# winddori2002/DEX-TTS

Hardware: AMD Instinct MI355X
Metric: mel-frames/s at n_timesteps=50, 80-ch mel (sampler only); RTF (higher is better)
Workload: dtype bf16; 1 GPU; gedex_b1: gedex_lj B=1/GPU T=512 n_timesteps=50 (BASELINE.json configs[1]); global_batch=1, frames=512, hipgraph=False, parallelism=1 GPU

## Files before the change

dex_tts_amd/csrc/dex_api.hip:

```cpp
#include <hip/hip_runtime.h>
#include <cstdlib>

#include <cmath>
#include <cstdarg>
#include <atomic>
#include <cstdio>
#include <mutex>
#include <cstring>
#include <map>
#include <unordered_map>
#include <string_view>
#include <string>
#include <vector>

#include "../../include/dex_amd.h"
#include "kernels.h"
#include "weight_store.h"

using namespace dex;

namespace dex {
namespace {
const char* const KNOB_NAMES[] = {
    "DEX_CONV_STREAM", "DEX_CONV_PP", "DEX_CONV_SKIP_DEAD", "DEX_H_BF16", "DEX_ATTN_SEPARATE", "DEX_ATTN_Q64", "DEX_ATTN_Q64_TAIL", "DEX_ATTN_Q64_HALF", "DEX_DIT_XCDS", "DEX_ATTN_GENERIC", "DEX_RES2", "DEX_LP_INTER", "DEX_DIT_CHAIN",
    "DEX_DIT_CLUSTER", "DEX_DIT_CLUSTER_LOCAL", "DEX_ATTN_X_LP", "DEX_RES_X_LP", "DEX_CAT_LP", "DEX_XCD_MAP", "DEX_DEBUG_DROP_HANDOFF", "DEX_PATCH_FUSED",
    "DEX_CONV_DOWN", "DEX_CONVT_UP", "DEX_DEBUG_PLAN",
    "DEX_ATTN_SHARED_W8", "DEX_CONVT_MT", "DEX_CONVT_WGS", "DEX_CONV_DOWN_WGS", "DEX_CONV_REGW", "DEX_CONV_REGW_RES", "DEX_CONV_SMALL_MAX", "DEX_CONV_TH8",
    "DEX_CONV_W8", "DEX_DWCONV_CAP", "DEX_FINAL_CAP", "DEX_FIRST_CAP", "DEX_FIRST_MFMA", "DEX_GEMM_NWALK", "DEX_NWALK_SPLIT", "DEX_NWALK_BM", "DEX_POS_COL", "DEX_POS_COL_MIN",
    "DEX_POS_CT", "DEX_REGW_MIN_TILES", "DEX_REGW_WGS", "DEX_ROWCHAIN64", "DEX_ROWCHAIN64A", "DEX_TIV_CAP", "DEX_TV_CHAIN", "DEX_TIV_FOLD", "DEX_LINATTN_NSUB", "DEX_TV_FOLD", "DEX_OUT2_MIN", "DEX_NWALK_DMA",
    "DEX_LINATTN_HEADWAVES", "DEX_LINATTN_OUT2_HW", "DEX_CONV_ROUND1", "DEX_CONV_RESIDENT", "DEX_KVCTX_ROWS", "DEX_OUT2_ROWS", "DEX_PE_TOK", "DEX_NWALK_SMALL"};
constexpr int N_KNOBS = (int)(sizeof(KNOB_NAMES) / sizeof(KNOB_NAMES[0]));
int knob_parse(const char* e) {
    if (!e) return KNOB_UNSET;
    char* end = nullptr;
    const long v = strtol(e, &end, 10);
    if (end == e) {
        static bool warned = false;
        if (!warned) { warned = true; fprintf(stderr, "libdexamd: ignoring a DEX_* knob whose value '%s' is not an integer\n", e); }
        return KNOB_UNSET;
    }
    return (int)v;
}
struct KnobSnapshot {
    int v[N_KNOBS];
    KnobSnapshot() { for (int i = 0; i < N_KNOBS; ++i) v[i] = knob_parse(getenv(KNOB_NAMES[i])); }
};
thread_local const KnobSnapshot* t_knobs = nullptr;
struct WsplitScope {
    bool prev;
    explicit WsplitScope(bool on) : prev(g_lp_wsplit) { g_lp_wsplit = on; }
    ~WsplitScope() { g_lp_wsplit = prev; }
};
struct KnobScope {
    const KnobSnapshot* prev;
    explicit KnobScope(const KnobSnapshot* k) : prev(t_knobs) { t_knobs = k; }
    ~KnobScope() { t_knobs = prev; }
};
}
static int knob_index(const char* name) {
    static const std::unordered_map<std::string_view, int> idx = [] {
        std::unordered_map<std::string_view, int> m;
        for (int i = 0; i < N_KNOBS; ++i) m.emplace(KNOB_NAMES[i], i);
        return m;
// ... 506 lines not shown
        build_mel_constants(basis, filt);
        DEX_HIPCHK(x, hipMalloc((void**)&x->mel_basis, basis.size() * sizeof(float)));
        DEX_HIPCHK(x, hipMalloc((void**)&x->mel_filt, filt.size() * sizeof(float)));
        DEX_HIPCHK(x, hipMemcpy(x->mel_basis, basis.data(), basis.size() * sizeof(float), hipMemcpyHostToDevice));
        DEX_HIPCHK(x, hipMemcpy(x->mel_filt, filt.data(), filt.size() * sizeof(float), hipMemcpyHostToDevice));
    }
    if (x->alloc_rc != DEX_OK) return x->alloc_rc;
    DEX_HIPCHK(x, hipStreamSynchronize(st));
    DEX_HIPCHK(x, hipGetLastError());
    x->finalized = true;
    return DEX_OK;
}

namespace {

constexpr int SCAL_STRIDE = 8;
constexpr int LA_CHUNK = 512;
constexpr int POS_SPLIT = 8;

struct Dims { int B, T, Tr, Ts, n_steps; };

struct StageBuf {
    int H, W, C, mask_ws; long npix;
    float *h1, *a1, *h2, *rbuf, *r0out, *r1out;
    float *qkv, *pm, *ps, *pc, *weff, *ctxn; void* mbf; int nchunks, nblk_fused;
    float* attn_out; int attn_ld, attn_coff;
    float* ds_out;
};

struct Plan {
    Dims d;
    float *sig2, *scal, *t_unet, *t_dit, *tmp_u, *temb, *c_tmp, *c_emb, *fin_mod;
    std::vector<float*> tadd_down, tadd_up, ada;
    float *adap_tmp, *t_adap, *t_sty, *tv_k0, *tv_v0, *sap_m, *sap_s, *ref_mean, *ref_std;
    float *spk_tmp, *spk_plane;
    int* step; int* step_tab; gnfix_t* stats; long stats_bytes; int n_gn;
    float* xbuf;
    float *xprime, *dbuf, *hsig, *htab;
    float *that, *hstep, *ncoef;
    std::vector<StageBuf> down, up;
    std::vector<float*> cat;
    void* cat16;
    float *up_out, *hF;
    int Hm, Wm, Hf, Wt, N;
    float *pe0, *emb, *emb_pad, *pos_part, *tok, *xn, *qkv, *ao, *att_ml, *hmlp, *dbg_tok;
    float* xslab; unsigned* xflag; size_t xflag_bytes;
    int xlocal;
    void *qh, *kh, *vt, *qh2, *kh2, *vt2; int Npad; size_t vt_bytes;
    float *tv_keys, *tv_K, *tv_V, *tv_q, *tv_ao, *tv_out, *tiv_out, *tv_weff, *tv_beff; gnfix_t *tv_stats, *tiv_stats; void* tv_wbf;
    float* tiv_aff;
    void *tv_kp, *tv_vtp; int tv_nkpad;
    float *tv_G, *tv_Vp, *tv_g0, *tv_v0p, *tv_xmean;
    float* xin;
    size_t bytes;
};

__global__ __launch_bounds__(256) void zero_fill_kernel(uint4* p16, size_t n16, unsigned char* tail, int ntail) {
    const uint4 z = make_uint4(0u, 0u, 0u, 0u);
    for (size_t i = (size_t)blockIdx.x * 256 + threadIdx.x; i < n16; i += (size_t)gridDim.x * 256) p16[i] = z;
    if (blockIdx.x == 0 && (int)threadIdx.x < ntail) tail[threadIdx.x] = 0;
}
static void zero_fill(void* p, size_t bytes, hipStream_t st) {
    if (!p || !bytes) return;
    const size_t n16 = bytes / 16;
    size_t blocks = (n16 + 255) / 256; if (blocks > 1024) blocks = 1024; if (blocks < 1) blocks = 1;
    hipLaunchKernelGGL(zero_fill_kernel, dim3((unsigned)blocks), dim3(256), 0, st, reinterpret_cast<uint4*>(p), n16,
                       reinterpret_cast<unsigned char*>(p) + n16 * 16, (int)(bytes - n16 * 16));
// ... 25 lines not shown
    if (g_xcd_map.load(std::memory_order_acquire) >= 0) return;
    std::lock_guard<std::mutex> lk(g_xcd_probe_mutex);
    if (g_xcd_map.load(std::memory_order_relaxed) >= 0) return;
    if (knob_off("DEX_DIT_CLUSTER_LOCAL")) { g_xcd_map.store(0, std::memory_order_release); return; }
    unsigned* d = nullptr;
    if (hipMalloc(&d, 256 * sizeof(unsigned)) != hipSuccess) { (void)hipGetLastError(); g_xcd_map.store(0, std::memory_order_release); return; }
    bool ok = hipFuncSetAttribute(reinterpret_cast<const void*>(&xcc_probe_kernel), hipFuncAttributeMaxDynamicSharedMemorySize, 65536) == hipSuccess;
    unsigned h[256];
    for (int rep = 0; rep < 3 && ok; ++rep) {
        const int nb = rep == 0 ? 256 : rep == 1 ? 96 : 192;
        hipLaunchKernelGGL(xcc_probe_kernel, dim3(nb), dim3(512), 65536, 0, d);
        ok = hipMemcpy(h, d, nb * sizeof(unsigned), hipMemcpyDeviceToHost) == hipSuccess;
        for (int b = 8; b < nb && ok; ++b) ok = h[b] == h[b & 7];
    }
    hipFree(d);
    g_xcd_map.store(ok ? 1 : 0, std::memory_order_release);
}
extern "C" int dex_debug_xcd_local() { xcd_map_probe(); return g_xcd_map.load(); }

void make_plan(const DexCtx* x, const Dims& d, void* ws, Plan& P) {
    const DexConfig& c = x->cfg;
    Arena A; A.base = (char*)ws; A.dry = (ws == nullptr);
    A.trace = knob_set("DEX_DEBUG_PLAN") ? 1 : 0;
    P.d = d;
    const int n = d.n_steps, dim = c.dim, hid = c.dit_hidden, mid = mid_dim(c), B = d.B;
    P.sig2 = A.f(64);
    P.scal = A.f((size_t)n * SCAL_STRIDE); P.t_unet = A.f((size_t)n * dim); P.t_dit = A.f((size_t)n * 256);
    P.tmp_u = A.f((size_t)n * 4 * dim); P.temb = A.f((size_t)n * dim);
    P.c_tmp = A.f((size_t)n * hid); P.c_emb = A.f((size_t)n * hid); P.fin_mod = A.f((size_t)n * 2 * hid);
    P.tadd_down.clear(); P.tadd_up.clear(); P.ada.clear();
    for (int i = 0; i < c.n_stages; ++i) for (int r = 0; r < 2; ++r) P.tadd_down.push_back(A.f((size_t)n * stage_dim(c, i)));
    for (int j = 0; j < c.n_stages - 1; ++j) for (int r = 0; r < 2; ++r) P.tadd_up.push_back(A.f((size_t)n * stage_dim(c, c.n_stages - 2 - j)));
    for (int k = 0; k < c.dit_depth; ++k) P.ada.push_back(A.f((size_t)n * 6 * hid));
    P.adap_tmp = P.t_adap = P.t_sty = P.tv_k0 = P.tv_v0 = P.sap_m = P.sap_s = P.ref_mean = P.ref_std = nullptr;
    if (c.variant == DEX_VARIANT_DEX) {
        P.adap_tmp = A.f((size_t)n * dim); P.t_adap = A.f((size_t)n * 2 * dim); P.t_sty = A.f((size_t)n * 2 * dim);
        P.tv_k0 = A.f((size_t)n * mid); P.tv_v0 = A.f((size_t)n * mid);
        P.sap_m = A.f((size_t)n * B * mid); P.sap_s = A.f((size_t)n * B * mid);
        P.ref_mean = A.f((size_t)B * 8 * mid); P.ref_std = A.f((size_t)B * 8 * mid);
    }
    P.spk_tmp = P.spk_plane = nullptr;
    if (c.n_spks > 1) { P.spk_tmp = A.f((size_t)B * 4 * c.spk_emb_dim); P.spk_plane = A.f((size_t)B * c.n_feats); }
    P.step = (int*)A.take(256);
    P.step_tab = (int*)A.take((size_t)(n + 1) * sizeof(int));
    P.n_gn = 4 * c.n_stages + 4 * (c.n_stages - 1) + 1;
    P.stats_bytes = (long)P.n_gn * B * 8 * GN_SLOTS * 2 * sizeof(gnfix_t);
    P.stats = (gnfix_t*)A.take(2 * P.stats_bytes);
    P.xbuf = A.f((size_t)B * 80 * d.T);
    P.xprime = A.f((size_t)B * 80 * d.T); P.dbuf = A.f((size_t)B * 80 * d.T);
    P.hsig = A.f((size_t)n + 2); P.htab = A.f((size_t)n + 2);
    P.that = A.f((size_t)n + 2); P.hstep = A.f((size_t)n + 2); P.ncoef = A.f((size_t)n + 2);
    P.cat.assign(c.n_stages - 1, nullptr);
    P.cat16 = nullptr;
    if (c.n_stages == 2) P.cat16 = A.take((size_t)B * (c.n_feats >> 1) * (d.T >> 1) * 2 * stage_dim(c, 1) * 2);
    for (int j = 0; j < c.n_stages - 1; ++j) {
        const int i = c.n_stages - 1 - j;
        P.cat[j] = A.f((size_t)B * (c.n_feats >> i) * (d.T >> i) * 2 * stage_dim(c, i));
    }
    auto stage = [&](int H, int W, int C, int mws) {
        StageBuf s{};
        s.H = H; s.W = W; s.C = C; s.mask_ws = mws; s.npix = (long)H * W;
        const size_t e = (size_t)B * s.npix;
        s.h1 = A.f(e * C); s.a1 = A.f(e * C); s.h2 = A.f(e * C); s.rbuf = A.f(e * C); s.r0out = A.f(e * C); s.r1out = A.f(e * C);
        s.qkv = A.f(e * 384);
        s.nchunks = (int)((s.npix + LA_CHUNK - 1) / LA_CHUNK);
        s.nblk_fused = (int)((s.npix + 127) / 128);
        s.pm = A.f((size_t)B * 4 * s.nblk_fused * 32); s.ps = A.f((size_t)B * 4 * s.nblk_fused * 32);
        s.pc = A.f((size_t)B * 4 * s.nblk_fused * 1024); s.weff = A.f((size_t)B * 128 * C);
        s.ctxn = A.f((size_t)B * 4096); s.mbf = A.take((size_t)B * C * 128 * 2);
// ... 688 lines not shown
                    ConvTUpP u{};
                    u.X = s.attn_out; u.a_lp = g.a_lp; u.ldx = s.C; u.xb = (long)s.H * s.W * s.C; u.x_coff = 0; u.H = s.H; u.W = s.W;
                    for (int par = 0; par < 4; ++par) u.Wfrag[par] = x->up_us_w[j][par].frag[x->lpi()].p;
                    u.bias = x->up_us_b[j];
                    u.Y = dst; u.c_lp = g.c_lp; u.ldy = ldd; u.y_coff = 0;
                    u.inmask = mask; u.inmask_ws = s.mask_ws; u.mask_bstride = P.d.T; u.B = B;
                    const double M = 4.0 * s.H * s.W * B;
                    run("upsample_convT", 2.0 * M * s.C * 4 * s.C, M * s.C * (g.c_lp ? 2.0 : 4.0) + 0.25 * M * s.C * (g.a_lp ? 2.0 : 4.0),
                        [&] { launch_convt_up(u, x->precision, st); });
                } else gemm("upsample_convT", g);
            }
        }
        tap("up_out", P.up_out, (long)B * 80 * P.d.T, c.dim, c.dim);
        TD U{P.up_out, c.dim, 0, c.dim, up_out_lp ? lpk : 0};
        gnfix_t* stf = next_stats();
        const bool hfb = h_bf16() && fast_conv(c.dim, c.dim);
        conv3x3("conv3x3", U, 80, P.d.T, 1, true, x->fin_w, x->fin_b, c.dim, P.hF, stf, nullptr, nullptr, nullptr, false, hfb);
        FinalGP f{};
        f.x_bf16 = hfb ? x->lp_kind() : 0;
        f.X = P.hF; f.xb = 80L * P.d.T * c.dim; f.npix = 80 * P.d.T; f.W = P.d.T; f.C = c.dim; f.groups = 8; f.stats = stf;
        f.gamma = x->fin_g; f.beta = x->fin_be; f.mask = mask; f.mask_bstride = P.d.T; f.wfc = x->fconv_w; f.bfc = x->fconv_b;
        f.xcur = xcur; f.denoised = denoised; f.xnext = xnext; f.scal = P.scal; f.scal_stride = SCAL_STRIDE; f.step = sp; f.row_bstride = rbs; f.B = B;
        f.zero_ptr = reinterpret_cast<float*>(stats_other); f.zero_n = P.stats_bytes / (long)sizeof(float);
        f.poison = P.xflag ? reinterpret_cast<const int*>(P.xflag + (P.xflag_bytes - sizeof(int)) / sizeof(unsigned)) : nullptr;
        f.mode = up.mode; f.htab = up.htab; f.dbuf = P.dbuf; f.xhat = P.xbuf;
        f.gtab = up.gtab; f.xstate = up.xstate; f.xin_next = up.xin_next;
        FinalMP fm{};
        static_cast<FinalP&>(fm) = f;
        fm.mtab = up.mtab; fm.dprev_in = up.dprev_in; fm.dprev_out = up.dprev_out;
        run("final_conv_euler", 14.0 * 80 * P.d.T * c.dim * B, 80.0 * P.d.T * ((hfb ? 2.0 : 4.0) * c.dim + 12.0) * B,
            [&] { if (up.mtab) launch_final_multistep(fm, st); else if (up.gtab) launch_final_general(f, st); else launch_final(f, st); });
    }

    void prepare(const float* sigmas_dev, int n, bool levels = false) {
        const DexConfig& c = x->cfg;
        const int dim = c.dim, hid = c.dit_hidden, B = P.d.B, mid = mid_dim(c);
        auto R = [&](const std::string& k) { return x->raw.at(k).p; };
        auto lin = [&](const float* X, int ldx, int rows, int K, const std::string& w, bool bias, int N, float* Y, int ai, int ao) {
            SmallLinP s{X, ldx, rows, K, R(w + ".weight"), bias ? R(w + ".bias") : nullptr, N, Y, N, ai, ao};
            run("cond_mlp", 2.0 * rows * K * N, 4.0 * K * N, [&] { launch_small_linear(s, st); });
        };
        if (P.tv_stats) zero_fill(P.tv_stats, (size_t)B * mid_dim(c) * IN_SLOTS * 2 * 2 * sizeof(gnfix_t), st);
        if (P.xflag) zero_fill(P.xflag, P.xflag_bytes, st);
        zero_fill(P.vt, P.vt_bytes, st);
        zero_fill(P.vt2, P.vt_bytes, st);
        CondPrepP cp{sigmas_dev, n, c.pe_scale, dim, P.scal, SCAL_STRIDE, P.t_unet, P.t_dit, levels ? 1 : 0};
        run("cond_prep", 0, 0, [&] { launch_cond_prep(cp, st); });
        lin(P.t_unet, dim, n, dim, "mlp.0", true, 4 * dim, P.tmp_u, 0, 1);
        lin(P.tmp_u, 4 * dim, n, 4 * dim, "mlp.2", true, dim, P.temb, 0, 0);
        for (int i = 0; i < c.n_stages; ++i)
            for (int r = 0; r < 2; ++r)
                lin(P.temb, dim, n, dim, "downs." + std::to_string(i) + "." + std::to_string(r) + ".mlp.1", true, stage_dim(c, i), P.tadd_down[2 * i + r], 1, 0);
        for (int j = 0; j < c.n_stages - 1; ++j)
            for (int r = 0; r < 2; ++r)
                lin(P.temb, dim, n, dim, "ups." + std::to_string(j) + "." + std::to_string(r) + ".mlp.1", true, stage_dim(c, c.n_stages - 2 - j), P.tadd_up[2 * j + r], 1, 0);
        lin(P.t_dit, 256, n, 256, "vit.t_embedder.mlp.0", true, hid, P.c_tmp, 0, 2);
        lin(P.c_tmp, hid, n, hid, "vit.t_embedder.mlp.2", true, hid, P.c_emb, 0, 0);
        for (int k = 0; k < c.dit_depth; ++k)
            lin(P.c_emb, hid, n, hid, "vit.blocks." + std::to_string(k) + ".adaLN_modulation.1", true, 6 * hid, P.ada[k], 2, 0);
        lin(P.c_emb, hid, n, hid, "vit.final_layer.adaLN_modulation.1", true, 2 * hid, P.fin_mod, 2, 0);
        if (c.n_spks > 1) {
            lin(args->spk_dev, c.spk_emb_dim, B, c.spk_emb_dim, "spk_mlp.0", true, 4 * c.spk_emb_dim, P.spk_tmp, 0, 1);
            lin(P.spk_tmp, 4 * c.spk_emb_dim, B, 4 * c.spk_emb_dim, "spk_mlp.2", true, c.n_feats, P.spk_plane, 0, 0);
        }
        if (c.variant == DEX_VARIANT_DEX) {
            lin(P.t_unet, dim, n, dim, "mlp_adap.0", true, dim, P.adap_tmp, 0, 1);
            lin(P.adap_tmp, dim, n, dim, "mlp_adap.2", true, 2 * dim, P.t_adap, 0, 0);
            lin(P.t_unet, dim, n, dim, "mlp_adap_sty.0", true, dim, P.adap_tmp, 0, 1);
            lin(P.adap_tmp, dim, n, dim, "mlp_adap_sty.2", true, 2 * dim, P.t_sty, 0, 0);
            lin(P.t_sty, mid, n, mid, "tv_adaptor.w_k", false, mid, P.tv_k0, 0, 0);
            lin(P.t_sty, mid, n, mid, "tv_adaptor.w_v", false, mid, P.tv_v0, 0, 0);
            const int L = args->n_ref;
            for (int j = 0; j < L; ++j)
                run("ref_stats", 0, 4.0 * B * mid * args->Tr, [&] {
                    launch_row_stats(args->ref_skips_dev[j], B, mid, args->Tr, 1e-5f, P.ref_mean + (long)j * mid, P.ref_std + (long)j * mid, (long)L * mid, st);
                });
            SapP sm{P.t_adap, 2 * dim, 0, n, P.ref_mean, L, mid, R("tiv_adaptor.mean_sap.W.weight"), R("tiv_adaptor.mean_sap.W.bias"), P.sap_m, B};
            SapP ss{P.t_adap, 2 * dim, 0, n, P.ref_std, L, mid, R("tiv_adaptor.std_sap.W.weight"), R("tiv_adaptor.std_sap.W.bias"), P.sap_s, B};
            run("sap_pool", 0, 0, [&] { launch_sap(sm, st); launch_sap(ss, st); });
            run("sty_transpose", 0, 8.0 * B * mid * args->Ts, [&] { launch_transpose_cl(args->sty_dev, P.tv_keys, B, mid, args->Ts, 0, (long)args->Ts * mid, st); });
            for (int which = 0; which < 2; ++which) {
                float* dst = which ? P.tv_V : P.tv_K;
                IGemmP g = base_gemm(P.tv_keys, mid, 0, 1, args->Ts, mid, which ? x->tv_wv : x->tv_wk, mid, nullptr, dst + mid, mid, 0);
                g.c_bstride = (long)(args->Ts + 1) * mid;
                gemm("tv_kv", g);
            }
            if (tv_chain_on()) {
                TvKvPrepP kp{P.tv_K, P.tv_V, (long)(args->Ts + 1) * mid, args->Ts + 1, P.tv_nkpad, P.tv_kp, P.tv_vtp, B};
                run("tv_kv_operands", 0, 12.0 * B * (args->Ts + 1) * mid, [&] { launch_tv_kv_prep(kp, x->precision, st); });
            }
            if (tv_fold_on()) {
                const long kvb = (long)(args->Ts + 1) * mid;
                for (int which = 0; which < 2; ++which) {
                    IGemmP g = base_gemm((which ? P.tv_V : P.tv_K) + mid, mid, 0, 1, args->Ts, mid, which ? x->tv_wl.f32 : x->tv_wq_raw, mid, nullptr,
                                         (which ? P.tv_Vp : P.tv_G) + mid, mid, 0);
                    g.a_bstride = kvb; g.c_bstride = kvb;
                    gemm("tv_fold_kv", g);
                    IGemmP t = base_gemm(which ? P.tv_v0 : P.tv_k0, mid, 0, 1, n, mid, which ? x->tv_wl.f32 : x->tv_wq_raw, mid, nullptr, which ? P.tv_v0p : P.tv_g0, mid, 0);
                    t.B = 1;
                    gemm("tv_fold_time_rows", t);
                }
                TvKvPrepP kp{P.tv_G, P.tv_Vp, kvb, args->Ts + 1, P.tv_nkpad, P.tv_kp, P.tv_vtp, B};
                run("tv_fold_operands", 0, 6.0 * B * (args->Ts + 1) * mid, [&] { launch_tv_vfrag_prep(kp, x->precision, st); });
            }
// ... 40 lines not shown

struct SamplerKind {
    const DexSamplerTables* tb;
    bool heun, multistep, churn, scaled;
    int n, E;
    explicit SamplerKind(const DexSampleArgs* a)
        : tb(a->tables), heun(a->solver == DEX_SOLVER_HEUN), multistep(a->solver == DEX_SOLVER_DPMPP_2M), churn(tb ? (tb->flags & DEX_TABLES_CHURN) != 0 : a->S_churn > 0.f),
          scaled(tb && (tb->flags & DEX_TABLES_SCALED) != 0), n(a->n_steps), E(tb ? tb->n_rows : dex_num_evals(a->n_steps, a->solver)) {}

    Eval eval(const Plan& P, int e) const {
        if (multistep) return {P.xbuf, P.xbuf, {0, nullptr, nullptr, nullptr, nullptr, tb->coef_dev, e == 0 ? nullptr : P.dbuf, P.dbuf}, -1};
        const int i = heun ? e / 2 : e;
        const bool corrector = heun && (e & 1);
        const bool predictor = heun && !corrector && i < n - 1;
        const int mode = corrector ? 2 : predictor ? 1 : 0, noise_step = (churn && !corrector) ? i : -1;
        float* x = corrector ? P.xprime : P.xbuf;
        float* xout = predictor ? P.xprime : P.xbuf;
        if (!tb) return {x, xout, {mode, heun ? P.htab : churn ? P.hstep : nullptr}, noise_step};
        float* xin_next = (scaled && (predictor || (!churn && i < n - 1))) ? P.xin : nullptr;
        return {scaled ? P.xin : x, xout, {mode, nullptr, tb->coef_dev, x, xin_next}, noise_step};
    }
};

int enqueue_sampler(DexCtx* x, const DexSampleArgs* a, hipStream_t st) {
    const SamplerKind k(a);
    const DexSamplerTables* tb = k.tb;
    const int n = k.n, E = k.E;
    Plan P; Dims d{a->B, a->T, a->Tr, a->Ts, E};
    make_plan(x, d, a->workspace_dev, P);
    Runner R{x, P, st, a->mask_dev, a->mu_dev, P.xbuf, a, false};
    const long nx = (long)a->B * 80 * a->T;
    float* xin = k.scaled ? P.xin : nullptr;
    auto coef = [&](int e) { return tb->coef_dev + (long)e * DEX_TABLE_EVAL_COLS; };
    if (tb) {
        R.prepare(tb->sigma_dev, E);
    } else {
        if (k.heun || k.churn) launch_churn_tables(a->sigmas_dev, n, a->S_churn, a->S_min, a->S_max, a->S_noise, P.that, P.hstep, P.ncoef, st);
        if (k.heun) launch_heun_expand(P.that, P.hstep, n, P.hsig, P.htab, st);
        R.prepare(k.heun ? P.hsig : k.churn ? P.that : a->sigmas_dev, E);
    }
    R.run("init_scale", 0, 8.0 * nx, [&] {
        if (tb) launch_ablation_init(a->z_dev, P.xbuf, tb->step_dev + 2, k.churn ? nullptr : xin, coef(0) + 1, nx, st);
        else launch_scale_copy(a->z_dev, P.xbuf, nx, a->sigmas_dev, st);
    });
    gnfix_t* arena[2] = {P.stats, P.stats + P.stats_bytes / (long)sizeof(gnfix_t)};
    zero_fill(P.stats, 2 * P.stats_bytes, st);
    for (int e = 0; e < E; ++e) {
        const Eval ev = k.eval(P, e);
        const int i = ev.noise_step;
        R.sp = e; R.stats_base = arena[e & 1]; R.stats_other = arena[(e + 1) & 1];
        if (i >= 0 && tb)
            R.run("churn_noise", 3.0 * nx, 16.0 * nx, [&] {
                launch_ablation_churn(P.xbuf, a->noise_dev ? a->noise_dev + (long)i * nx : nullptr, tb->step_dev + (long)i * DEX_TABLE_STEP_COLS,
                                      xin, coef(e) + 1, nx, st);
            });
        else if (i >= 0)
            R.run("churn_noise", 2.0 * nx, 12.0 * nx, [&] { launch_add_noise(P.xbuf, a->noise_dev + (long)i * nx, P.ncoef + i, nx, st); });
        R.xcur = ev.xin; R.up = ev.up;
        R.step(nullptr, ev.xout);
    }
    R.run("copy_out", 0, 8.0 * nx, [&] { launch_scale_copy(P.xbuf, a->out_dev, nx, nullptr, st); });
    return DEX_OK;
}

struct CallScope {
    const KnobSnapshot knobs;
    const KnobScope knob_scope{&knobs};
    const WsplitScope wsplit_scope;
    explicit CallScope(DexCtx* x) : wsplit_scope(x->precision == DEX_PREC_FP16X2) { xcd_map_probe(); x->last_xerr = nullptr; }
};

std::vector<uint64_t> graph_key(const DexSampleArgs* a, int precision, hipStream_t st, const KnobSnapshot& knobs) {
    std::vector<uint64_t> key = {(uint64_t)a->B, (uint64_t)a->T, (uint64_t)a->Tr, (uint64_t)a->Ts, (uint64_t)a->n_steps, (uint64_t)a->solver,
                                 (uint64_t)precision, (uint64_t)a->n_ref, (uint64_t)(uintptr_t)st,
                                 (uint64_t)(uintptr_t)a->z_dev, (uint64_t)(uintptr_t)a->mu_dev, (uint64_t)(uintptr_t)a->mask_dev,
                                 (uint64_t)(uintptr_t)a->sigmas_dev, (uint64_t)(uintptr_t)a->spk_dev, (uint64_t)(uintptr_t)a->sty_dev,
                                 (uint64_t)(uintptr_t)a->sty_lengths_dev, (uint64_t)(uintptr_t)a->out_dev, (uint64_t)(uintptr_t)a->workspace_dev,
                                 (uint64_t)(uintptr_t)(a->S_churn > 0.f ? a->noise_dev : nullptr)};
    key.push_back((uint64_t)g_xcd_gen.load(std::memory_order_acquire));
// ... 300 lines not shown
```

dex_tts_amd/csrc/kernels.h:

```cpp
#pragma once
#include <hip/hip_runtime.h>
#include <stdint.h>

namespace dex {

constexpr int KNOB_UNSET = -2147483647 - 1;
int knob(const char* name);
inline int knob_or(const char* name, int dflt) { const int v = knob(name); return v == KNOB_UNSET ? dflt : v; }
inline bool knob_off(const char* name) { return knob(name) == 0; }
inline bool knob_set(const char* name) { return knob(name) != KNOB_UNSET; }
inline int device_cus() {
    static const int n = [] { int dev = 0, v = 0; (void)hipGetDevice(&dev); (void)hipDeviceGetAttribute(&v, hipDeviceAttributeMultiprocessorCount, dev); return v > 0 ? v : 256; }();
    return n;
}

constexpr int GN_SLOTS = 32;
typedef long long gnfix_t;

extern thread_local const char* g_last_symbol;

constexpr int PREC_FP32 = 0, PREC_BF16 = 1, PREC_FP16 = 2, PREC_FP16X2 = 3;
inline bool prec_wsplit(int precision) { return precision == PREC_FP16X2; }
extern thread_local bool g_lp_wsplit;
inline bool prec_is_lp(int precision) { return precision != PREC_FP32; }
// ... 224 lines not shown
                     int xcd_map;
                     int tail_g = 0, tail_ks = 0;
                     int half_g = 0, half_n = 0; };
void launch_attention_direct(const AttnDirectP& p, int precision, hipStream_t st);
bool attention_direct_batch_regime(int N, int B);
int attention_direct_ksplit(int N, int B);
void launch_attention_q64(const AttnDirectP& p, int precision, hipStream_t st);
int attention_q64_ksplit(int N, int B, int max_split);
void attention_q64_plan(int N, int B, int max_split, int* ks, int* tail_g, int* tail_ks);
bool attention_q64_half_plan(int N, int B, int* half_g, int* half_n);
void launch_dit_rowchain(const DitChainP& p, int precision, hipStream_t st);
void launch_pack_lp_frag(const float* src, void* dst, int K, int N, int precision, hipStream_t st);
void launch_pack_lp_frag_nk(const float* src, void* dst, int K, int N, int precision, hipStream_t st);

struct AttnP { const float* Q; int ldq; long qb; const float* K; int ldk; long kb; const float* V; int ldv; long vb;
               float* O; int ldo; long ob; int Nq, Nk; const int* kv_len; int kv_len_add; int heads; float scale; int B;
               int ksplit; long o_sstride; float* ml;
               long long* dbg;
               int head_dim;
               int force_generic;
               int o_lp; };
inline bool dit_sep64_small_n(int N, int B) {
    if (N < 512 || N >= 1024) return false;
    const long t = (long)B * ((N + 63) / 64), r = (t + 255) / 256;
    return t >= 256 && t * 100 >= r * 256 * 65;
}
bool attention_lp_shared_form(int Nq, int heads, int B, int ksplit);
bool attention_head_dim_supported(int hd);
void launch_attention(const AttnP& p, int precision, hipStream_t st);

struct SmallLinP { const float* X; int ldx; int rows; int K; const float* W; const float* bias; int N;
                   float* Y; int ldy; int act_in; int act_out; };
void launch_small_linear(const SmallLinP& p, hipStream_t st);

struct CondPrepP { const float* sigmas; int n; float pe_scale; int dim; float* scal; int scal_stride;
                   float* t_unet; float* t_dit;
                   int no_next = 0; };
void launch_cond_prep(const CondPrepP& p, hipStream_t st);

void launch_scale_copy(const float* src, float* dst, long n, const float* scal_ptr, hipStream_t st);
void launch_step_reset(int* step, hipStream_t st);
void launch_step_inc(int* step, hipStream_t st);
void launch_iota(int* dst, int n, hipStream_t st);
void launch_permute4(const float* src, float* dst, int d0, int d1, int d2, int d3, int p0, int p1, int p2, int p3,
                     hipStream_t st);
void launch_f32_residual_lp(const float* src, float* dst, long n, int precision, hipStream_t st);
void launch_f32_to_lp(const float* src, void* dst, long n, int precision, hipStream_t st);
void launch_pack_lp_nk(const float* src, void* dst, int K, int N, int precision, hipStream_t st);
void launch_spk_plane(const float* spk_out, float* plane, int B, int F, hipStream_t st);

void launch_row_stats(const float* X, int B, int C, int len, float eps, float* mean, float* std, long out_bstride, hipStream_t st);
constexpr int IN_SLOTS = GN_SLOTS;
struct InStatsP { const float* X; int ld; long bstride; int npix; int C; gnfix_t* stats; int B;
                  const float* mask; int mask_ws; long mask_bstride; int W; };
void launch_in_stats(const InStatsP& p, hipStream_t st);
struct SapP { const float* t_tok; int t_ld; int t_coff; int nsteps; const float* stats; int L; int C;
              const float* w; const float* bias; float* out; int B; };
void launch_sap(const SapP& p, hipStream_t st);
struct InFoldP { const gnfix_t* stats; int npix; float eps; const float* Wq; int C; float* Weff; float* beff; int B;
                 void* Wbf; int lp; int split = 0; };
void launch_in_fold(const InFoldP& p, hipStream_t st);
struct TivApplyP { const float* X; int ld; long xb; float* Y; int ldy; long yb; int npix; int C; const gnfix_t* stats;
                   float eps; const float* s_tab; const float* m_tab; int step; int B;
                   int row_bstride = 0; };
void launch_tiv_apply(const TivApplyP& p, hipStream_t st);
void launch_tiv_coef(const TivApplyP& p, float* aff, hipStream_t st);
struct TvRow0P { const float* k0; const float* v0; int step; float* K; float* V; long kvb; int C; int B;
                 float* zero_ptr; long zero_n;
                 void* Kp = nullptr; void* VTp = nullptr; int NkPad = 0; int lp_kind = 0;
                 int row_bstride = 0; };
void launch_tv_row0(const TvRow0P& p, hipStream_t st);
// ... 81 lines not shown
```

dex_tts_amd/csrc/unet_elem.hip:

```cpp
#include "kernels.h"
#include "bf16_util.h"
#include <cstdlib>

namespace dex {

__device__ __forceinline__ float mish_f(float x) {
    if (x > 20.f) return x;
    const float e = __expf(x);
    const float n = e * (e + 2.f);
    return x * (n * __builtin_amdgcn_rcpf(n + 2.f));
}
__device__ __forceinline__ float silu_f(float x) { return x * __builtin_amdgcn_rcpf(1.f + __expf(-x)); }


__device__ __forceinline__ void gn_mean_rstd(const gnfix_t* stats, int b, int groups, float* smean, float* srstd, int tid) {
    if (tid < groups * GN_SLOTS) {
        const int g = tid / GN_SLOTS;
        const longlong2 v = *reinterpret_cast<const longlong2*>(stats + (((long)b * groups + g) * GN_SLOTS + (tid % GN_SLOTS)) * 2);
        long long s1 = v.x, s2 = v.y;
        gn_slots_reduce<GN_SLOTS>(s1, s2);
        if ((tid % GN_SLOTS) == 0) gn_moments(s1, s2, 1e-5, smean[g], srstd[g]);
    }
}

// ... 595 lines not shown
    hipLaunchKernelGGL(final_kernel<FinalGP>, dim3((unsigned)final_blocks(p), p.B), dim3(256), 0, st, p);
}
__global__ void ablation_churn_kernel(float* x, const float* noise, const float* rk, float* xin, const float* s, long n) {
    const float r = rk[0], k = rk[1];
    const float sv = xin ? *s : 1.f;
    for (long i = (long)blockIdx.x * blockDim.x + threadIdx.x; i < n; i += (long)gridDim.x * blockDim.x) {
        float v = __fmul_rn(r, x[i]);
        if (noise) v = __fadd_rn(v, __fmul_rn(k, noise[i]));
        x[i] = v;
        if (xin) xin[i] = __fdiv_rn(v, sv);
    }
}
void launch_final_multistep(const FinalMP& p, hipStream_t st) {
    hipLaunchKernelGGL(final_kernel<FinalMP>, dim3((unsigned)final_blocks(p), p.B), dim3(256), 0, st, p);
}
void launch_ablation_churn(float* x, const float* noise, const float* rk, float* xin, const float* s, long n, hipStream_t st) {
    long blocks = (n + 255) / 256; if (blocks > 2048) blocks = 2048;
    hipLaunchKernelGGL(ablation_churn_kernel, dim3((unsigned)blocks), dim3(256), 0, st, x, noise, rk, xin, s, n);
}
__global__ void ablation_init_kernel(const float* z, float* x, const float* c0, float* xin, const float* s, long n) {
    const float c = *c0;
    const float sv = xin ? *s : 1.f;
    for (long i = (long)blockIdx.x * blockDim.x + threadIdx.x; i < n; i += (long)gridDim.x * blockDim.x) {
        const float v = __fmul_rn(z[i], c);
        x[i] = v;
        if (xin) xin[i] = __fdiv_rn(v, sv);
    }
}
void launch_ablation_init(const float* z, float* x, const float* c0, float* xin, const float* s, long n, hipStream_t st) {
    long blocks = (n + 255) / 256; if (blocks > 2048) blocks = 2048;
    hipLaunchKernelGGL(ablation_init_kernel, dim3((unsigned)blocks), dim3(256), 0, st, z, x, c0, xin, s, n);
}

__global__ void cond_prep_kernel(const CondPrepP p) {
    const int i = blockIdx.x;
    const int k = threadIdx.x;
    const float sigma = p.sigmas[i], sigma_next = p.no_next ? 0.f : p.sigmas[i + 1];
    const float sd = 0.5f;
    const float c_noise = logf(sigma) / 4.f;
    if (k == 0) {
        float* sc = p.scal + (long)i * p.scal_stride;
        const float s2 = sigma * sigma + sd * sd;
        sc[0] = sigma; sc[1] = sigma_next;
        sc[2] = 1.f / sqrtf(s2);
        sc[3] = __fmul_rn(__frcp_rn(s2), sd * sd);
        sc[4] = sigma * sd / sqrtf(s2);
        sc[5] = c_noise;
    }
    const int half = p.dim / 2;
    if (k < half) {
        const float e = (float)(log(10000.0) / (double)(half - 1));
        const float f = expf((float)k * -e);
        const float a = p.pe_scale * c_noise * f;
        p.t_unet[(long)i * p.dim + k] = sinf(a);
        p.t_unet[(long)i * p.dim + half + k] = cosf(a);
    }
    if (k < 128) {
        const float f = expf((float)(-log(10000.0)) * (float)k / 128.f);
        const float a = c_noise * f;
        p.t_dit[(long)i * 256 + k] = cosf(a);
        p.t_dit[(long)i * 256 + 128 + k] = sinf(a);
    }
}
void launch_cond_prep(const CondPrepP& p, hipStream_t st) {
    hipLaunchKernelGGL(cond_prep_kernel, dim3(p.n), dim3(128), 0, st, p);
}

__global__ __launch_bounds__(256) void small_linear_kernel(const SmallLinP p) {
    const int wave = (blockIdx.x * 256 + threadIdx.x) >> 6, lane = threadIdx.x & 63;
    if (wave >= p.N) return;
    const float* w = p.W + (long)wave * p.K;
    const float bias = p.bias ? p.bias[wave] : 0.f;
    const int r0 = blockIdx.y * 8;
    float acc[8];
#pragma unroll
    for (int j = 0; j < 8; ++j) acc[j] = 0.f;
    for (int k = lane; k < p.K; k += 64) {
        const float wk = w[k];
#pragma unroll
        for (int j = 0; j < 8; ++j) {
            const int r = min(r0 + j, p.rows - 1);
            float v = p.X[(long)r * p.ldx + k];
            if (p.act_in == 1) v = mish_f(v); else if (p.act_in == 2) v = silu_f(v);
            acc[j] = fmaf(v, wk, acc[j]);
        }
    }
#pragma unroll
    for (int j = 0; j < 8; ++j) {
        float a = acc[j];
        for (int o = 32; o > 0; o >>= 1) a += __shfl_xor(a, o);
        if (lane == 0 && r0 + j < p.rows) {
            float y = a + bias;
            if (p.act_out == 1) y = mish_f(y); else if (p.act_out == 2) y = silu_f(y);
            p.Y[(long)(r0 + j) * p.ldy + wave] = y;
        }
    }
}
void launch_small_linear(const SmallLinP& p, hipStream_t st) {
    hipLaunchKernelGGL(small_linear_kernel, dim3((p.N * 64 + 255) / 256, (p.rows + 7) / 8), dim3(256), 0, st, p);
}

__global__ void scale_copy_kernel(const float* src, float* dst, long n, const float* scal) {
    const float s = scal ? *scal : 1.f;
    for (long i = (long)blockIdx.x * blockDim.x + threadIdx.x; i < n; i += (long)gridDim.x * blockDim.x) dst[i] = src[i] * s;
}
void launch_scale_copy(const float* src, float* dst, long n, const float* scal_ptr, hipStream_t st) {
    long blocks = (n + 255) / 256; if (blocks > 2048) blocks = 2048;
    hipLaunchKernelGGL(scale_copy_kernel, dim3((unsigned)blocks), dim3(256), 0, st, src, dst, n, scal_ptr);
}
__global__ void iota_kernel(int* d, int n) { const int i = blockIdx.x * blockDim.x + threadIdx.x; if (i < n) d[i] = i; }
void launch_iota(int* dst, int n, hipStream_t st) { hipLaunchKernelGGL(iota_kernel, dim3((n + 255) / 256), dim3(256), 0, st, dst, n); }
__global__ void step_reset_kernel(int* s) { *s = 0; }
__global__ void step_inc_kernel(int* s) { *s = *s + 1; }
void launch_step_reset(int* step, hipStream_t st) { hipLaunchKernelGGL(step_reset_kernel, dim3(1), dim3(1), 0, st, step); }
void launch_step_inc(int* step, hipStream_t st) { hipLaunchKernelGGL(step_inc_kernel, dim3(1), dim3(1), 0, st, step); }

__global__ void permute4_kernel(const float* src, float* dst, int d0, int d1, int d2, int d3, int p0, int p1, int p2, int p3) {
    const long n = (long)d0 * d1 * d2 * d3;
    const int sd[4] = {d0, d1, d2, d3};
    const long ss[4] = {(long)d1 * d2 * d3, (long)d2 * d3, (long)d3, 1};
    const int pm[4] = {p0, p1, p2, p3};
    for (long i = (long)blockIdx.x * blockDim.x + threadIdx.x; i < n; i += (long)gridDim.x * blockDim.x) {
        long rem = i, off = 0;
        for (int a = 3; a >= 0; --a) {
            const int dim = sd[pm[a]];
            const int idx = (int)(rem % dim);
            rem /= dim;
            off += idx * ss[pm[a]];
        }
        dst[i] = src[off];
    }
}
// ... 42 lines not shown
```

Measured before the change: 29630 mel-frames/s.

## Batch conditioning MLP launches and fuse per-call zero-fills, cond prep, init scale

Conditioning linears in prepare() are grouped by dependency level and issued as one multi-job small-linear kernel per level, with weights held in registers when K<=256. The separate zero-fills, cond_prep and initial noise scaling are merged into a single call_begin kernel. This cuts the per-call launch count in the fixed setup before the sampler loop. A second scratch buffer keeps the two adaptor MLP chains from racing inside a level. The path is on by default and can be disabled with DEX_COND_BATCH.

Result: no change. 29670 mel-frames/s (median of 4 runs) (+0.1%).

```diff
diff --git a/dex_tts_amd/csrc/dex_api.hip b/dex_tts_amd/csrc/dex_api.hip
--- a/dex_tts_amd/csrc/dex_api.hip
+++ b/dex_tts_amd/csrc/dex_api.hip
@@ -28,7 +28,8 @@
     "DEX_ATTN_SHARED_W8", "DEX_CONVT_MT", "DEX_CONVT_WGS", "DEX_CONV_DOWN_WGS", "DEX_CONV_REGW", "DEX_CONV_REGW_RES", "DEX_CONV_SMALL_MAX", "DEX_CONV_TH8",
     "DEX_CONV_W8", "DEX_DWCONV_CAP", "DEX_FINAL_CAP", "DEX_FIRST_CAP", "DEX_FIRST_MFMA", "DEX_GEMM_NWALK", "DEX_NWALK_SPLIT", "DEX_NWALK_BM", "DEX_POS_COL", "DEX_POS_COL_MIN",
     "DEX_POS_CT", "DEX_REGW_MIN_TILES", "DEX_REGW_WGS", "DEX_ROWCHAIN64", "DEX_ROWCHAIN64A", "DEX_TIV_CAP", "DEX_TV_CHAIN", "DEX_TIV_FOLD", "DEX_LINATTN_NSUB", "DEX_TV_FOLD", "DEX_OUT2_MIN", "DEX_NWALK_DMA",
-    "DEX_LINATTN_HEADWAVES", "DEX_LINATTN_OUT2_HW", "DEX_CONV_ROUND1", "DEX_CONV_RESIDENT", "DEX_KVCTX_ROWS", "DEX_OUT2_ROWS", "DEX_PE_TOK", "DEX_NWALK_SMALL"};
+    "DEX_LINATTN_HEADWAVES", "DEX_LINATTN_OUT2_HW", "DEX_CONV_ROUND1", "DEX_CONV_RESIDENT", "DEX_KVCTX_ROWS", "DEX_OUT2_ROWS", "DEX_PE_TOK", "DEX_NWALK_SMALL",
+    "DEX_COND_BATCH"};
 constexpr int N_KNOBS = (int)(sizeof(KNOB_NAMES) / sizeof(KNOB_NAMES[0]));
 int knob_parse(const char* e) {
     if (!e) return KNOB_UNSET;
@@ -601,7 +602,7 @@
     Dims d;
     float *sig2, *scal, *t_unet, *t_dit, *tmp_u, *temb, *c_tmp, *c_emb, *fin_mod;
     std::vector<float*> tadd_down, tadd_up, ada;
-    float *adap_tmp, *t_adap, *t_sty, *tv_k0, *tv_v0, *sap_m, *sap_s, *ref_mean, *ref_std;
+    float *adap_tmp, *adap_tmp2, *t_adap, *t_sty, *tv_k0, *tv_v0, *sap_m, *sap_s, *ref_mean, *ref_std;
     float *spk_tmp, *spk_plane;
     int* step; int* step_tab; gnfix_t* stats; long stats_bytes; int n_gn;
     float* xbuf;
@@ -693,9 +694,9 @@
     for (int i = 0; i < c.n_stages; ++i) for (int r = 0; r < 2; ++r) P.tadd_down.push_back(A.f((size_t)n * stage_dim(c, i)));
     for (int j = 0; j < c.n_stages - 1; ++j) for (int r = 0; r < 2; ++r) P.tadd_up.push_back(A.f((size_t)n * stage_dim(c, c.n_stages - 2 - j)));
     for (int k = 0; k < c.dit_depth; ++k) P.ada.push_back(A.f((size_t)n * 6 * hid));
-    P.adap_tmp = P.t_adap = P.t_sty = P.tv_k0 = P.tv_v0 = P.sap_m = P.sap_s = P.ref_mean = P.ref_std = nullptr;
+    P.adap_tmp = P.adap_tmp2 = P.t_adap = P.t_sty = P.tv_k0 = P.tv_v0 = P.sap_m = P.sap_s = P.ref_mean = P.ref_std = nullptr;
     if (c.variant == DEX_VARIANT_DEX) {
-        P.adap_tmp = A.f((size_t)n * dim); P.t_adap = A.f((size_t)n * 2 * dim); P.t_sty = A.f((size_t)n * 2 * dim);
+        P.adap_tmp = A.f((size_t)n * dim); P.adap_tmp2 = A.f((size_t)n * dim); P.t_adap = A.f((size_t)n * 2 * dim); P.t_sty = A.f((size_t)n * 2 * dim);
         P.tv_k0 = A.f((size_t)n * mid); P.tv_v0 = A.f((size_t)n * mid);
         P.sap_m = A.f((size_t)n * B * mid); P.sap_s = A.f((size_t)n * B * mid);
         P.ref_mean = A.f((size_t)B * 8 * mid); P.ref_std = A.f((size_t)B * 8 * mid);
@@ -1450,44 +1451,72 @@
             [&] { if (up.mtab) launch_final_multistep(fm, st); else if (up.gtab) launch_final_general(f, st); else launch_final(f, st); });
     }
 
-    void prepare(const float* sigmas_dev, int n, bool levels = false) {
+    static bool cond_batch() { return !knob_off("DEX_COND_BATCH"); }
+    void prepare(const float* sigmas_dev, int n, bool levels = false, bool clear_stats = false, const float* z0 = nullptr, const float* sigma0 = nullptr) {
         const DexConfig& c = x->cfg;
         const int dim = c.dim, hid = c.dit_hidden, B = P.d.B, mid = mid_dim(c);
+        const bool batch = cond_batch();
         auto R = [&](const std::string& k) { return x->raw.at(k).p; };
-        auto lin = [&](const float* X, int ldx, int rows, int K, const std::string& w, bool bias, int N, float* Y, int ai, int ao) {
+        std::vector<SmallLinP> jobs[3];
+        double fl[3] = {0, 0, 0}, by[3] = {0, 0, 0};
+        auto lin = [&](int level, const float* X, int ldx, int rows, int K, const std::string& w, bool bias, int N, float* Y, int ai, int ao) {
             SmallLinP s{X, ldx, rows, K, R(w + ".weight"), bias ? R(w + ".bias") : nullptr, N, Y, N, ai, ao};
-            run("cond_mlp", 2.0 * rows * K * N, 4.0 * K * N, [&] { launch_small_linear(s, st); });
+            if (!batch) { run("cond_mlp", 2.0 * rows * K * N, 4.0 * K * N, [&] { launch_small_linear(s, st); }); return; }
+            jobs[level - 1].push_back(s); fl[level - 1] += 2.0 * rows * K * N; by[level - 1] += 4.0 * K * N;
         };
-        if (P.tv_stats) zero_fill(P.tv_stats, (size_t)B * mid_dim(c) * IN_SLOTS * 2 * 2 * sizeof(gnfix_t), st);
-        if (P.xflag) zero_fill(P.xflag, P.xflag_bytes, st);
-        zero_fill(P.vt, P.vt_bytes, st);
-        zero_fill(P.vt2, P.vt_bytes, st);
+        const size_t tv_stats_bytes = P.tv_stats ? (size_t)B * mid_dim(c) * IN_SLOTS * 2 * 2 * sizeof(gnfix_t) : 0;
         CondPrepP cp{sigmas_dev, n, c.pe_scale, dim, P.scal, SCAL_STRIDE, P.t_unet, P.t_dit, levels ? 1 : 0};
-        run("cond_prep", 0, 0, [&] { launch_cond_prep(cp, st); });
-        lin(P.t_unet, dim, n, dim, "mlp.0", true, 4 * dim, P.tmp_u, 0, 1);
-        lin(P.tmp_u, 4 * dim, n, 4 * dim, "mlp.2", true, dim, P.temb, 0, 0);
+        if (batch) {
+            CallBeginP cb{};
+            auto zero = [&](void* p, size_t bytes) { if (p && bytes) cb.zero[cb.n_zero++] = {p, bytes}; };
+            zero(P.tv_stats, tv_stats_bytes);
+            zero(P.xflag, P.xflag_bytes);
+            zero(P.vt, P.vt_bytes);
+            zero(P.vt2, P.vt_bytes);
+            if (clear_stats) zero(P.stats, 2 * (size_t)P.stats_bytes);
+            cb.cp = cp;
+            cb.z = z0; cb.x0 = P.xbuf; cb.nx = (long)B * 80 * P.d.T; cb.sigma0 = sigma0;
+            run("call_begin", 0, z0 ? 8.0 * cb.nx : 0, [&] { launch_call_begin(cb, st); });
+        } else {
+            if (P.tv_stats) zero_fill(P.tv_stats, tv_stats_bytes, st);
+            if (P.xflag) zero_fill(P.xflag, P.xflag_bytes, st);
+            zero_fill(P.vt, P.vt_bytes, st);
+            zero_fill(P.vt2, P.vt_bytes, st);
+            run("cond_prep", 0, 0, [&] { launch_cond_prep(cp, st); });
+        }
+        lin(1, P.t_unet, dim, n, dim, "mlp.0", true, 4 * dim, P.tmp_u, 0, 1);
+        lin(2, P.tmp_u, 4 * dim, n, 4 * dim, "mlp.2", true, dim, P.temb, 0, 0);
         for (int i = 0; i < c.n_stages; ++i)
             for (int r = 0; r < 2; ++r)
-                lin(P.temb, dim, n, dim, "downs." + std::to_string(i) + "." + std::to_string(r) + ".mlp.1", true, stage_dim(c, i), P.tadd_down[2 * i + r], 1, 0);
+                lin(3, P.temb, dim, n, dim, "downs." + std::to_string(i) + "." + std::to_string(r) + ".mlp.1", true, stage_dim(c, i), P.tadd_down[2 * i + r], 1, 0);
         for (int j = 0; j < c.n_stages - 1; ++j)
             for (int r = 0; r < 2; ++r)
-                lin(P.temb, dim, n, dim, "ups." + std::to_string(j) + "." + std::to_string(r) + ".mlp.1", true, stage_dim(c, c.n_stages - 2 - j), P.tadd_up[2 * j + r], 1, 0);
-        lin(P.t_dit, 256, n, 256, "vit.t_embedder.mlp.0", true, hid, P.c_tmp, 0, 2);
-        lin(P.c_tmp, hid, n, hid, "vit.t_embedder.mlp.2", true, hid, P.c_emb, 0, 0);
+                lin(3, P.temb, dim, n, dim, "ups." + std::to_string(j) + "." + std::to_string(r) + ".mlp.1", true, stage_dim(c, c.n_stages - 2 - j), P.tadd_up[2 * j + r], 1, 0);
+        lin(1, P.t_dit, 256, n, 256, "vit.t_embedder.mlp.0", true, hid, P.c_tmp, 0, 2);
+        lin(2, P.c_tmp, hid, n, hid, "vit.t_embedder.mlp.2", true, hid, P.c_emb, 0, 0);
         for (int k = 0; k < c.dit_depth; ++k)
-            lin(P.c_emb, hid, n, hid, "vit.blocks." + std::to_string(k) + ".adaLN_modulation.1", true, 6 * hid, P.ada[k], 2, 0);
-        lin(P.c_emb, hid, n, hid, "vit.final_layer.adaLN_modulation.1", true, 2 * hid, P.fin_mod, 2, 0);
+            lin(3, P.c_emb, hid, n, hid, "vit.blocks." + std::to_string(k) + ".adaLN_modulation.1", true, 6 * hid, P.ada[k], 2, 0);
+        lin(3, P.c_emb, hid, n, hid, "vit.final_layer.adaLN_modulation.1", true, 2 * hid, P.fin_mod, 2, 0);
         if (c.n_spks > 1) {
-            lin(args->spk_dev, c.spk_emb_dim, B, c.spk_emb_dim, "spk_mlp.0", true, 4 * c.spk_emb_dim, P.spk_tmp, 0, 1);
-            lin(P.spk_tmp, 4 * c.spk_emb_dim, B, 4 * c.spk_emb_dim, "spk_mlp.2", true, c.n_feats, P.spk_plane, 0, 0);
+            lin(1, args->spk_dev, c.spk_emb_dim, B, c.spk_emb_dim, "spk_mlp.0", true, 4 * c.spk_emb_dim, P.spk_tmp, 0, 1);
+            lin(2, P.spk_tmp, 4 * c.spk_emb_dim, B, 4 * c.spk_emb_dim, "spk_mlp.2", true, c.n_feats, P.spk_plane, 0, 0);
         }
         if (c.variant == DEX_VARIANT_DEX) {
-            lin(P.t_unet, dim, n, dim, "mlp_adap.0", true, dim, P.adap_tmp, 0, 1);
-            lin(P.adap_tmp, dim, n, dim, "mlp_adap.2", true, 2 * dim, P.t_adap, 0, 0);
-            lin(P.t_unet, dim, n, dim, "mlp_adap_sty.0", true, dim, P.adap_tmp, 0, 1);
-            lin(P.adap_tmp, dim, n, dim, "mlp_adap_sty.2", true, 2 * dim, P.t_sty, 0, 0);
-            lin(P.t_sty, mid, n, mid, "tv_adaptor.w_k", false, mid, P.tv_k0, 0, 0);
-            lin(P.t_sty, mid, n, mid, "tv_adaptor.w_v", false, mid, P.tv_v0, 0, 0);
+            float* sty_tmp = batch ? P.adap_tmp2 : P.adap_tmp;
+            lin(1, P.t_unet, dim, n, dim, "mlp_adap.0", true, dim, P.adap_tmp, 0, 1);
+            lin(2, P.adap_tmp, dim, n, dim, "mlp_adap.2", true, 2 * dim, P.t_adap, 0, 0);
+            lin(1, P.t_unet, dim, n, dim, "mlp_adap_sty.0", true, dim, sty_tmp, 0, 1);
+            lin(2, sty_tmp, dim, n, dim, "mlp_adap_sty.2", true, 2 * dim, P.t_sty, 0, 0);
+            lin(3, P.t_sty, mid, n, mid, "tv_adaptor.w_k", false, mid, P.tv_k0, 0, 0);
+            lin(3, P.t_sty, mid, n, mid, "tv_adaptor.w_v", false, mid, P.tv_v0, 0, 0);
+        }
+        for (int l = 0; l < 3; ++l)
+            for (size_t first = 0; first < jobs[l].size(); first += SMALL_LIN_BATCH) {
+                const int cnt = (int)std::min<size_t>(jobs[l].size() - first, SMALL_LIN_BATCH);
+                const double share = (double)cnt / (double)jobs[l].size();
+                run("cond_mlp", fl[l] * share, by[l] * share, [&] { launch_small_linear_batch(jobs[l].data() + first, cnt, st); });
+            }
+        if (c.variant == DEX_VARIANT_DEX) {
             const int L = args->n_ref;
             for (int j = 0; j < L; ++j)
                 run("ref_stats", 0, 4.0 * B * mid * args->Tr, [&] {
@@ -1594,19 +1623,20 @@
     const long nx = (long)a->B * 80 * a->T;
     float* xin = k.scaled ? P.xin : nullptr;
     auto coef = [&](int e) { return tb->coef_dev + (long)e * DEX_TABLE_EVAL_COLS; };
+    const bool batch = Runner::cond_batch(), x0_in_begin = batch && !tb;
     if (tb) {
-        R.prepare(tb->sigma_dev, E);
+        R.prepare(tb->sigma_dev, E, false, batch);
     } else {
         if (k.heun || k.churn) launch_churn_tables(a->sigmas_dev, n, a->S_churn, a->S_min, a->S_max, a->S_noise, P.that, P.hstep, P.ncoef, st);
         if (k.heun) launch_heun_expand(P.that, P.hstep, n, P.hsig, P.htab, st);
-        R.prepare(k.heun ? P.hsig : k.churn ? P.that : a->sigmas_dev, E);
-    }
-    R.run("init_scale", 0, 8.0 * nx, [&] {
+        R.prepare(k.heun ? P.hsig : k.churn ? P.that : a->sigmas_dev, E, false, batch, batch ? a->z_dev : nullptr, a->sigmas_dev);
+    }
+    if (!x0_in_begin) R.run("init_scale", 0, 8.0 * nx, [&] {
         if (tb) launch_ablation_init(a->z_dev, P.xbuf, tb->step_dev + 2, k.churn ? nullptr : xin, coef(0) + 1, nx, st);
         else launch_scale_copy(a->z_dev, P.xbuf, nx, a->sigmas_dev, st);
     });
     gnfix_t* arena[2] = {P.stats, P.stats + P.stats_bytes / (long)sizeof(gnfix_t)};
-    zero_fill(P.stats, 2 * P.stats_bytes, st);
+    if (!batch) zero_fill(P.stats, 2 * P.stats_bytes, st);
     for (int e = 0; e < E; ++e) {
         const Eval ev = k.eval(P, e);
         const int i = ev.noise_step;
diff --git a/dex_tts_amd/csrc/kernels.h b/dex_tts_amd/csrc/kernels.h
--- a/dex_tts_amd/csrc/kernels.h
+++ b/dex_tts_amd/csrc/kernels.h
@@ -280,11 +280,19 @@
 struct SmallLinP { const float* X; int ldx; int rows; int K; const float* W; const float* bias; int N;
                    float* Y; int ldy; int act_in; int act_out; };
 void launch_small_linear(const SmallLinP& p, hipStream_t st);
+constexpr int SMALL_LIN_BATCH = 16;
+struct SmallLinBatchP { SmallLinP job[SMALL_LIN_BATCH]; int wg0[SMALL_LIN_BATCH + 1]; int n; int gpw; };
+void launch_small_linear_batch(const SmallLinP* jobs, int n, hipStream_t st);
 
 struct CondPrepP { const float* sigmas; int n; float pe_scale; int dim; float* scal; int scal_stride;
                    float* t_unet; float* t_dit;
                    int no_next = 0; };
 void launch_cond_prep(const CondPrepP& p, hipStream_t st);
+constexpr int CALL_BEGIN_ZEROS = 5;
+struct CallBeginP { struct Zero { void* p; size_t bytes; } zero[CALL_BEGIN_ZEROS]; int n_zero; int zero_blocks;
+                    CondPrepP cp;
+                    const float* z; float* x0; long nx; const float* sigma0; int x0_blocks; };
+void launch_call_begin(CallBeginP p, hipStream_t st);
 
 void launch_scale_copy(const float* src, float* dst, long n, const float* scal_ptr, hipStream_t st);
 void launch_step_reset(int* step, hipStream_t st);
diff --git a/dex_tts_amd/csrc/unet_elem.hip b/dex_tts_amd/csrc/unet_elem.hip
--- a/dex_tts_amd/csrc/unet_elem.hip
+++ b/dex_tts_amd/csrc/unet_elem.hip
@@ -651,9 +651,7 @@
     hipLaunchKernelGGL(ablation_init_kernel, dim3((unsigned)blocks), dim3(256), 0, st, z, x, c0, xin, s, n);
 }
 
-__global__ void cond_prep_kernel(const CondPrepP p) {
-    const int i = blockIdx.x;
-    const int k = threadIdx.x;
+__device__ __forceinline__ void cond_prep_row(const CondPrepP& p, const int i, const int k) {
     const float sigma = p.sigmas[i], sigma_next = p.no_next ? 0.f : p.sigmas[i + 1];
     const float sd = 0.5f;
     const float c_noise = logf(sigma) / 4.f;
@@ -681,8 +679,36 @@
         p.t_dit[(long)i * 256 + 128 + k] = sinf(a);
     }
 }
+__global__ void cond_prep_kernel(const CondPrepP p) { cond_prep_row(p, blockIdx.x, threadIdx.x); }
 void launch_cond_prep(const CondPrepP& p, hipStream_t st) {
     hipLaunchKernelGGL(cond_prep_kernel, dim3(p.n), dim3(128), 0, st, p);
+}
+
+__global__ __launch_bounds__(256) void call_begin_kernel(const CallBeginP p) {
+    const int b = blockIdx.x, t = threadIdx.x;
+    if (b < p.zero_blocks) {
+        const uint4 z = make_uint4(0u, 0u, 0u, 0u);
+        for (int r = 0; r < p.n_zero; ++r) {
+            uint4* p16 = reinterpret_cast<uint4*>(p.zero[r].p);
+            const size_t n16 = p.zero[r].bytes / 16;
+            for (size_t i = (size_t)b * 256 + t; i < n16; i += (size_t)p.zero_blocks * 256) p16[i] = z;
+            const int ntail = (int)(p.zero[r].bytes - n16 * 16);
+            if (b == 0 && t < ntail) reinterpret_cast<unsigned char*>(p.zero[r].p)[n16 * 16 + t] = 0;
+        }
+    } else if (b < p.zero_blocks + p.cp.n) {
+        if (t < 128) cond_prep_row(p.cp, b - p.zero_blocks, t);
+    } else {
+        const float s = *p.sigma0;
+        const long nb = p.x0_blocks;
+        for (long i = (long)(b - p.zero_blocks - p.cp.n) * 256 + t; i < p.nx; i += nb * 256) p.x0[i] = p.z[i] * s;
+    }
+}
+void launch_call_begin(CallBeginP p, hipStream_t st) {
+    size_t n16 = 0;
+    for (int r = 0; r < p.n_zero; ++r) n16 = std::max(n16, p.zero[r].bytes / 16);
+    p.zero_blocks = (int)std::min<size_t>(std::max<size_t>((n16 + 255) / 256, 1), 1024);
+    p.x0_blocks = p.z ? (int)std::min<long>((p.nx + 255) / 256, 2048) : 0;
+    hipLaunchKernelGGL(call_begin_kernel, dim3(p.zero_blocks + p.cp.n + p.x0_blocks), dim3(256), 0, st, p);
 }
 
 __global__ __launch_bounds__(256) void small_linear_kernel(const SmallLinP p) {
@@ -717,6 +743,69 @@
 }
 void launch_small_linear(const SmallLinP& p, hipStream_t st) {
     hipLaunchKernelGGL(small_linear_kernel, dim3((p.N * 64 + 255) / 256, (p.rows + 7) / 8), dim3(256), 0, st, p);
+}
+
+__device__ __forceinline__ void small_linear_fma(const SmallLinP& p, const int k, const int r0, const float wk, float (&acc)[8]) {
+#pragma unroll
+    for (int j = 0; j < 8; ++j) {
+        const int r = min(r0 + j, p.rows - 1);
+        float v = p.X[(long)r * p.ldx + k];
+        if (p.act_in == 1) v = mish_f(v); else if (p.act_in == 2) v = silu_f(v);
+        acc[j] = fmaf(v, wk, acc[j]);
+    }
+}
+__device__ __forceinline__ void small_linear_store(const SmallLinP& p, const int n, const int lane, const int r0, const float bias, const float (&acc)[8]) {
+#pragma unroll
+    for (int j = 0; j < 8; ++j) {
+        float a = acc[j];
+        for (int o = 32; o > 0; o >>= 1) a += __shfl_xor(a, o);
+        if (lane == 0 && r0 + j < p.rows) {
+            float y = a + bias;
+            if (p.act_out == 1) y = mish_f(y); else if (p.act_out == 2) y = silu_f(y);
+            p.Y[(long)(r0 + j) * p.ldy + n] = y;
+        }
+    }
+}
+__global__ __launch_bounds__(256) void small_linear_batch_kernel(const SmallLinBatchP b) {
+    int job = 0;
+    while (job + 1 < b.n && (int)blockIdx.x >= b.wg0[job + 1]) ++job;
+    const SmallLinP& p = b.job[job];
+    const int n = ((int)blockIdx.x - b.wg0[job]) * 4 + ((int)threadIdx.x >> 6), lane = threadIdx.x & 63;
+    if (n >= p.N || (int)blockIdx.y * b.gpw * 8 >= p.rows) return;
+    const float* wrow = p.W + (long)n * p.K;
+    const float bias = p.bias ? p.bias[n] : 0.f;
+    const bool resident = p.K <= 256;
+    float w[4];
+#pragma unroll
+    for (int i = 0; i < 4; ++i) w[i] = (resident && lane + 64 * i < p.K) ? wrow[lane + 64 * i] : 0.f;
+    const int r_begin = (int)blockIdx.y * b.gpw * 8, r_end = min(p.rows, r_begin + b.gpw * 8);
+    for (int r0 = r_begin; r0 < r_end; r0 += 8) {
+        float acc[8];
+#pragma unroll
+        for (int j = 0; j < 8; ++j) acc[j] = 0.f;
+        if (resident) {
+#pragma unroll
+            for (int i = 0; i < 4; ++i)
+                if (lane + 64 * i < p.K) small_linear_fma(p, lane + 64 * i, r0, w[i], acc);
+        } else {
+            for (int k = lane; k < p.K; k += 64) small_linear_fma(p, k, r0, wrow[k], acc);
+        }
+        small_linear_store(p, n, lane, r0, bias, acc);
+    }
+}
+void launch_small_linear_batch(const SmallLinP* jobs, int n, hipStream_t st) {
+    SmallLinBatchP b{};
+    b.n = std::min(n, SMALL_LIN_BATCH);
+    long waves = 0; int groups = 1;
+    for (int j = 0; j < b.n; ++j) {
+        b.job[j] = jobs[j]; b.wg0[j + 1] = b.wg0[j] + (jobs[j].N + 3) / 4;
+        waves += jobs[j].N; groups = std::max(groups, (jobs[j].rows + 7) / 8);
+    }
+    constexpr long RESIDENT_WAVES = 256 * 4 * 8;
+    b.gpw = 1;
+    while (b.gpw < groups && waves * ((groups + b.gpw - 1) / b.gpw) > RESIDENT_WAVES) ++b.gpw;
+    if (b.wg0[b.n] > 0)
+        hipLaunchKernelGGL(small_linear_batch_kernel, dim3(b.wg0[b.n], (groups + b.gpw - 1) / b.gpw), dim3(256), 0, st, b);
 }
 
 __global__ void scale_copy_kernel(const float* src, float* dst, long n, const float* scal) {
```
